# facebookresearch/D3GA

Hardware: AMD Instinct MI355X
Metric: fwd+bwd frames/sec @500k Gaussians 1920x1080 (higher is better)
Workload: dtype f32

## Files before the change

d3ga_amd/csrc/raster_pre.hip:

```cpp
#include "composite_common.h"
#include "raster_pre_body.h"

namespace d3ga {

constexpr int kShRow = 52;
constexpr int kShSlab = 64 * kShRow;
constexpr size_t kShLdsBytes = (size_t)(kBlock / 64) * kShSlab * sizeof(float);

__host__ __device__ __forceinline__ bool sh_staged(int M) { return M > 0 && (3 * M) % 4 == 0 && 3 * M <= 48; }

__device__ __forceinline__ void sh_slab_load(float *slab, const float *__restrict__ src, int rows, int M3, int lane) {
    const int nvec = rows * M3 / 4;
    for (int v = lane; v < nvec; v += 64) {
        const float4 x = reinterpret_cast<const float4 *>(src)[v];
        const int e = 4 * v, r = e / M3, c = e - r * M3;
        *reinterpret_cast<float4 *>(slab + r * kShRow + c) = x;
    }
}
__device__ __forceinline__ void sh_slab_store(const float *slab, float *__restrict__ dst, int rows, int M3, int lane) {
    const int nvec = rows * M3 / 4;
    for (int v = lane; v < nvec; v += 64) {
        const int e = 4 * v, r = e / M3, c = e - r * M3;
        reinterpret_cast<float4 *>(dst)[v] = *reinterpret_cast<const float4 *>(slab + r * kShRow + c);
    }
}

template <int ROWS>
struct ShRegs { float4 v[ROWS * 12 / 64]; };
template <int ROWS>
__device__ __forceinline__ ShRegs<ROWS> sh_rows48_load(const float *__restrict__ src, int lane) {
    ShRegs<ROWS> r;
#pragma unroll
    for (int k = 0; k < ROWS * 12 / 64; ++k) r.v[k] = reinterpret_cast<const float4 *>(src)[lane + 64 * k];
    return r;
}
template <int ROWS>
__device__ __forceinline__ void sh_rows48_to_slab(float *slab, const ShRegs<ROWS> &r, int lane) {
#pragma unroll
    for (int k = 0; k < ROWS * 12 / 64; ++k) {
        const int e = 4 * (lane + 64 * k), row = e / 48, c = e - row * 48;
        *reinterpret_cast<float4 *>(slab + row * kShRow + c) = r.v[k];
    }
}
template <int ROWS>
__device__ __forceinline__ void sh_rows48_store(const float *slab, float *__restrict__ dst, int lane) {
#pragma unroll
    for (int k = 0; k < ROWS * 12 / 64; ++k) {
        const int e = 4 * (lane + 64 * k), row = e / 48, c = e - row * 48;
        reinterpret_cast<float4 *>(dst)[lane + 64 * k] = *reinterpret_cast<const float4 *>(slab + row * kShRow + c);
    }
}

constexpr int kShPassRows = 32;
constexpr int kShHalfSlab = kShPassRows * kShRow;
constexpr size_t kShHalfLdsBytes = (size_t)(kBlock / 64) * kShHalfSlab * sizeof(float);

template <bool WANT_J>
__device__ __forceinline__ void staged_sh_colour(const d3ga_raster_params &prm, const float *__restrict__ means3D,
                                                 const float *__restrict__ shs, const float *__restrict__ campos,
                                                 float *s_sh, float acc[3], ShColJ &cj) {
    const int tid = threadIdx.x, lane = tid & 63, wave = tid >> 6;
    const int i = blockIdx.x * kBlock + tid;
    const int M3 = 3 * prm.M;
    float *slab = s_sh + wave * kShHalfSlab;
    const int row0 = blockIdx.x * kBlock + wave * 64;
    const int rows = min(64, prm.P - row0);
    const int nb = (prm.sh_degree + 1) * (prm.sh_degree + 1);
    float B[16];
    float dx = 0.f, dy = 0.f, dz = 1.f;
    if (WANT_J && i < prm.P) sh_view_dir(means3D, i, campos, dx, dy, dz);
    auto eval = [&](const float *row) __attribute__((always_inline)) {
        if (WANT_J) cj = sh_accumulate_jacobian(B, dx, dy, dz, row, nb, cj);
        else sh_accumulate(B, row, 0, 16, nb, acc);
    };
    if (M3 == 48 && rows == 64) {
        const float *src = shs + (size_t)48 * row0;
        const ShRegs<kShPassRows> h0 = sh_rows48_load<kShPassRows>(src, lane);
        const ShRegs<kShPassRows> h1 = sh_rows48_load<kShPassRows>(src + 48 * kShPassRows, lane);
        sh_view_basis(prm, means3D, i, campos, B);
        __builtin_amdgcn_wave_barrier();
        sh_rows48_to_slab<kShPassRows>(slab, h0, lane);
        __builtin_amdgcn_wave_barrier();
        if (lane / kShPassRows == 0) eval(slab + (lane % kShPassRows) * kShRow);
        __builtin_amdgcn_wave_barrier();
        sh_rows48_to_slab<kShPassRows>(slab, h1, lane);
        __builtin_amdgcn_wave_barrier();
        if (lane / kShPassRows == 1) eval(slab + (lane % kShPassRows) * kShRow);
        return;
    }
    if (i < prm.P) sh_view_basis(prm, means3D, i, campos, B);
    for (int h = 0; h < 2; ++h) {
        const int r = min(kShPassRows, rows - kShPassRows * h);
        __builtin_amdgcn_wave_barrier();
        if (r > 0) sh_slab_load(slab, shs + (size_t)M3 * (row0 + kShPassRows * h), r, M3, lane);
        __builtin_amdgcn_wave_barrier();
        if (i < prm.P && lane / kShPassRows == h) eval(slab + (lane % kShPassRows) * kShRow);
    }
}

struct TileRect { bool visible; int r0, r1, r2, r3; };
__device__ __forceinline__ TileRect view_tile_rect(const PreOut &o, int tile_row0) {
    const Splat &sp = o.sp;
    return TileRect{sp.visible, sp.rect[0], sp.rect[1] + tile_row0, sp.rect[2], sp.rect[3] + tile_row0};
}
__device__ __forceinline__ void write_geom_records(const GeomBuf &geom, int i, const PreOut &o, bool keep_cov, int tile_row0,
                                                   int32_t *__restrict__ radii, bool want_j, const ShColJ &cj) {
    const Splat &sp = o.sp;
    if (keep_cov) {
#pragma unroll
        for (int k = 0; k < 6; ++k) geom.cov3D[6 * (size_t)i + k] = o.c6[k];
    }
    radii[i] = sp.radius;
    geom.depth[i] = sp.depth;
    geom.rect[i] = sp.visible ? make_uint2((uint32_t)sp.rect[0] | ((uint32_t)(sp.rect[1] + tile_row0) << 16),
                                           (uint32_t)sp.rect[2] | ((uint32_t)(sp.rect[3] + tile_row0) << 16))
                              : make_uint2(0u, 0u);
    geom.conic_o[i] = make_float4(sp.conic[0], sp.conic[1], sp.conic[2], o.opacity);
    {
        const SplatCull sc = splat_cull(sp.conic[0], sp.conic[1], sp.conic[2], o.opacity);
        geom.xyh[i] = make_float4(sp.px, sp.py, sp.visible ? sc.hx : -1.0f, sc.hy);
    }
    geom.rgb_invd[i] = make_float4(o.rgb[0], o.rgb[1], o.rgb[2], sp.visible ? 1.0f / sp.depth : 0.f);
    geom.clamped[i] = o.clampmask;
    if (want_j) dcol_store(geom.dcol, geom.dcol_stride, i, cj);
}

__device__ __forceinline__ PreOut window_clip(PreOut o, int x0, int y0, int gx, int gy) {
    Splat &sp = o.sp;
    const int r0 = max(sp.rect[0], x0) - x0, r1 = max(sp.rect[1], y0) - y0;
    const int r2 = min(sp.rect[2], x0 + gx) - x0, r3 = min(sp.rect[3], y0 + gy) - y0;
    if (sp.visible && r2 > r0 && r3 > r1) { sp.rect[0] = r0; sp.rect[1] = r1; sp.rect[2] = r2; sp.rect[3] = r3; }
    else { sp.visible = false; sp.rect[0] = sp.rect[1] = sp.rect[2] = sp.rect[3] = 0; }
    return o;
}
__global__ void window_table_kernel(d3ga_raster_params prm, const float *__restrict__ campos, int views, int4 *__restrict__ table) {
    const int v = blockIdx.x * blockDim.x + threadIdx.x;
    if (v >= views) return;
    const ViewCam c = view_cam(prm, nullptr, nullptr, campos + (size_t)D3GA_CAMERA_SLOT_WINDOWED_FLOATS * v, true);
    table[v] = make_int4(c.ox, c.oy, c.W, c.H);
}

struct TileResv { TileWindow win; uint32_t base[kResvSlots]; };
__device__ __forceinline__ TileResv tile_reserve_issue(uint32_t *s_win, const TileRect &t, int gx, uint32_t *__restrict__ tile_count,
                                                       uint32_t *__restrict__ tile_count2, uint32_t *__restrict__ vis_part) {
    const int lane = threadIdx.x & 63;
    TileResv r;
    r.win = wave_tile_window(t.visible, t.r0, t.r1, t.r2, t.r3);
#pragma unroll
    for (int j = 0; j < kResvSlots; ++j) r.base[j] = 0u;
    const unsigned long long vis = __ballot(t.visible);
    if (lane == 0 && vis) atomicAdd(&vis_part[((blockIdx.x * (kBlock / 64) + (threadIdx.x >> 6)) % kVisParts) * kVisStride], (uint32_t)__popcll(vis));
    if (r.win.empty()) return r;
    if (r.win.fits()) {
        const int area = r.win.area();
        __builtin_amdgcn_wave_barrier();
#pragma unroll
        for (int j = 0; j < kResvSlots; ++j)
            if (lane + 64 * j < area) s_win[lane + 64 * j] = 0u;
        __builtin_amdgcn_wave_barrier();
        if (t.visible)
            for (int ty = t.r1; ty < t.r3; ++ty)
                for (int tx = t.r0; tx < t.r2; ++tx) atomicAdd(&s_win[(ty - r.win.y0) * r.win.w + (tx - r.win.x0)], 1u);
        __builtin_amdgcn_wave_barrier();
        const float inv_w = 1.0f / (float)r.win.w;
#pragma unroll
        for (int j = 0; j < kResvSlots; ++j) {
            const int k = lane + 64 * j;
            const uint32_t c = k < area ? s_win[k] : 0u;
            if (c) r.base[j] = atomicAdd(&tile_count[r.win.tile_of(k, gx, inv_w)], c);
        }
    } else {
        if (lane == 0) atomicOr(&vis_part[kUnresvWord], 1u);
        if (t.visible)
            for (int ty = t.r1; ty < t.r3; ++ty)
                for (int tx = t.r0; tx < t.r2; ++tx) atomicAdd(&tile_count2[ty * gx + tx], 1u);
    }
    return r;
}
__device__ __forceinline__ void tile_reserve_store(const TileResv &r, uint32_t *__restrict__ rec) {
    const int lane = threadIdx.x & 63;
    if (lane == 0)
        *reinterpret_cast<uint4 *>(rec) = make_uint4((uint32_t)r.win.x0 | ((uint32_t)r.win.y0 << 16), (uint32_t)r.win.w | ((uint32_t)r.win.h << 16), 0u, 0u);
    if (r.win.empty() || !r.win.fits()) return;
    const int area = r.win.area();
#pragma unroll
    for (int j = 0; j < kResvSlots; ++j)
        if (lane + 64 * j < area) rec[kResvHdr + lane + 64 * j] = r.base[j];
}

template <bool WIN>
__device__ __forceinline__ PreOut preprocess_view(const d3ga_raster_params &prm, const ViewCam &cam, int i, const float *means3D,
                                                    const float *sh_row, bool staged, const ShColJ &cj, bool pre, const float (&pc6)[6],
                                                    float pop, const float *colors_precomp, const float *opacities, const float *scales,
                                                    const float *rotations, const float *cov3D_precomp, int gx, int gy) {
    PreLoaded pl;
    pl.has_sh = staged; pl.has_c6 = pre;
    pl.sh[0] = cj.a0; pl.sh[1] = cj.a1; pl.sh[2] = cj.a2;
#pragma unroll
    for (int k = 0; k < 6; ++k) pl.c6[k] = pc6[k];
    pl.op = pop;
    PreOut o = preprocess_one(prm, cam, i, means3D, sh_row, colors_precomp, opacities, scales, rotations, cov3D_precomp, pl);
    if constexpr (WIN) o = window_clip(o, cam.ox / kTile, cam.oy / kTile, gx, gy);
    return o;
}

template <bool WANT_J, bool WIN>
__global__ __launch_bounds__(kBlock) void preprocess_kernel(
    d3ga_raster_params prm, const float *__restrict__ means3D, const float *__restrict__ shs,
    const float *__restrict__ colors_precomp, const float *__restrict__ opacities, const float *__restrict__ scales,
    const float *__restrict__ rotations, const float *__restrict__ cov3D_precomp, const float *__restrict__ viewmatrix,
    const float *__restrict__ projmatrix, const float *__restrict__ campos, GeomBuf geom,
    uint32_t *__restrict__ tile_count, uint32_t *__restrict__ tile_count2, uint32_t *__restrict__ vis_part,
    uint32_t *__restrict__ resv , int32_t *__restrict__ radii,
    int tile_row0 ) {
    const ViewCam cam = view_cam(prm, viewmatrix, projmatrix, campos, WIN);
    const int gx = (prm.W + kTile - 1) / kTile + (WIN ? 1 : 0), gy = (prm.H + kTile - 1) / kTile + 1;
    extern __shared__ __attribute__((aligned(16))) char smem[];
    float *s_sh = reinterpret_cast<float *>(smem);
    const int tid = threadIdx.x, wave = tid >> 6;
    const int i = blockIdx.x * kBlock + tid;
    const int M3 = 3 * prm.M;
    const bool staged = shs != nullptr && sh_staged(prm.M);
    uint32_t *s_win = reinterpret_cast<uint32_t *>(smem) + wave * (staged ? kShHalfSlab : kResvStride);
    float pc6[6] = {0.f, 0.f, 0.f, 0.f, 0.f, 0.f}, pop = 0.f;
    const bool pre = staged && cov3D_precomp != nullptr;
    if (pre && i < prm.P) {
#pragma unroll
        for (int k = 0; k < 6; ++k) pc6[k] = cov3D_precomp[6 * (size_t)i + k];
        pop = opacities[i];
    }
    ShColJ cj = {0.f, 0.f, 0.f, 0.f, 0.f, 0.f, 0.f, 0.f, 0.f, 0.f, 0.f, 0.f};
    float acc[3] = {0.f, 0.f, 0.f};
    if (staged) {
        staged_sh_colour<WANT_J>(prm, means3D, shs, campos, s_sh, acc, cj);
        if (!WANT_J) { cj.a0 = acc[0]; cj.a1 = acc[1]; cj.a2 = acc[2]; }
    }
    TileRect tr = {false, 0, 0, 0, 0};
    PreOut o = {};
    if (i < prm.P) {
        o = staged ? preprocess_view<WIN>(prm, cam, i, means3D, nullptr, true, cj, pre, pc6, pop, colors_precomp, opacities, scales,
                                          rotations, cov3D_precomp, gx, gy)
                   : preprocess_view<WIN>(prm, cam, i, means3D, shs ? shs + (size_t)M3 * i : nullptr, false, cj, false, pc6, pop,
                                          colors_precomp, opacities, scales, rotations, cov3D_precomp, gx, gy);
        tr = view_tile_rect(o, tile_row0);
    }
    const TileResv rs = tile_reserve_issue(s_win, tr, gx, tile_count, tile_count2, vis_part);
    if (i < prm.P) write_geom_records(geom, i, o, !cov3D_precomp, tile_row0, radii, WANT_J, cj);
    tile_reserve_store(rs, resv + (size_t)(blockIdx.x * (kBlock / 64) + wave) * kResvStride);
}

template <bool WANT_J, int KV>
__device__ __forceinline__ void staged_sh_colour_views(const d3ga_raster_params &prm, const float *__restrict__ means3D, size_t pv,
                                                       const float *__restrict__ shs, const ViewCams<KV> &cams, float *s_sh,
                                                       ShColJ (&cj)[KV]) {
    const int tid = threadIdx.x, lane = tid & 63, wave = tid >> 6;
    const int i = blockIdx.x * kBlock + tid;
    const int M3 = 3 * prm.M;
    float *slab = s_sh + wave * kShHalfSlab;
    const int row0 = blockIdx.x * kBlock + wave * 64;
    const int rows = min(64, prm.P - row0);
    const int nb = (prm.sh_degree + 1) * (prm.sh_degree + 1);
    auto eval = [&](const float *row) __attribute__((always_inline)) {
#pragma unroll
        for (int v = 0; v < KV; ++v) {
            float B[16];
            const float *mv = means3D + 3 * pv * v;
            if (WANT_J) {
                float dx, dy, dz;
                sh_view_dir(mv, i, cams.cp[v], dx, dy, dz);
                sh_basis(prm.sh_degree, dx, dy, dz, B);
                cj[v] = sh_accumulate_jacobian(B, dx, dy, dz, row, nb, cj[v]);
            } else {
                sh_view_basis(prm, mv, i, cams.cp[v], B);
                float acc[3] = {cj[v].a0, cj[v].a1, cj[v].a2};
                sh_accumulate(B, row, 0, 16, nb, acc);
                cj[v].a0 = acc[0]; cj[v].a1 = acc[1]; cj[v].a2 = acc[2];
            }
        }
    };
    if (M3 == 48 && rows == 64) {
        const float *src = shs + (size_t)48 * row0;
        const ShRegs<kShPassRows> h0 = sh_rows48_load<kShPassRows>(src, lane);
        const ShRegs<kShPassRows> h1 = sh_rows48_load<kShPassRows>(src + 48 * kShPassRows, lane);
        __builtin_amdgcn_wave_barrier();
        sh_rows48_to_slab<kShPassRows>(slab, h0, lane);
        __builtin_amdgcn_wave_barrier();
        if (lane / kShPassRows == 0) eval(slab + (lane % kShPassRows) * kShRow);
        __builtin_amdgcn_wave_barrier();
        sh_rows48_to_slab<kShPassRows>(slab, h1, lane);
        __builtin_amdgcn_wave_barrier();
        if (lane / kShPassRows == 1) eval(slab + (lane % kShPassRows) * kShRow);
        return;
    }
    for (int h = 0; h < 2; ++h) {
        const int r = min(kShPassRows, rows - kShPassRows * h);
        __builtin_amdgcn_wave_barrier();
        if (r > 0) sh_slab_load(slab, shs + (size_t)M3 * (row0 + kShPassRows * h), r, M3, lane);
        __builtin_amdgcn_wave_barrier();
        if (i < prm.P && lane / kShPassRows == h) eval(slab + (lane % kShPassRows) * kShRow);
    }
}

template <bool WANT_J, int KV>
__global__ __launch_bounds__(kBlock) void preprocess_views_kernel(
    d3ga_raster_params prm, const float *__restrict__ means3D, const float *__restrict__ shs,
    const float *__restrict__ colors_precomp, const float *__restrict__ opacities, const float *__restrict__ scales,
    const float *__restrict__ rotations, const float *__restrict__ cov3D_precomp, ViewCams<KV> cams, GeomBuf geom ,
    uint32_t *__restrict__ tile_count, uint32_t *__restrict__ tile_count2, uint32_t *__restrict__ vis_part,
    uint32_t *__restrict__ resv , int32_t *__restrict__ radii ,
    int tile_row0, int gyv, size_t pv ) {
    extern __shared__ __attribute__((aligned(16))) char smem[];
    float *s_sh = reinterpret_cast<float *>(smem);
    const int tid = threadIdx.x, wave = tid >> 6;
    const int i = blockIdx.x * kBlock + tid;
    uint32_t *s_win = reinterpret_cast<uint32_t *>(smem) + wave * kShHalfSlab;
    const size_t wpv = (size_t)gridDim.x * (kBlock / 64);
    float pc6[6] = {0.f, 0.f, 0.f, 0.f, 0.f, 0.f}, pop = 0.f;
    const bool pre = cov3D_precomp != nullptr && pv == 0;
    if (pre && i < prm.P) {
#pragma unroll
        for (int k = 0; k < 6; ++k) pc6[k] = cov3D_precomp[6 * (size_t)i + k];
        pop = opacities[i];
    }
    ShColJ cj[KV];
#pragma unroll
    for (int v = 0; v < KV; ++v) cj[v] = ShColJ{0.f, 0.f, 0.f, 0.f, 0.f, 0.f, 0.f, 0.f, 0.f, 0.f, 0.f, 0.f};
    staged_sh_colour_views<WANT_J, KV>(prm, means3D, pv, shs, cams, s_sh, cj);
    const int gx = (prm.W + kTile - 1) / kTile;
#pragma unroll
    for (int v = 0; v < KV; ++v) {
        TileRect tr = {false, 0, 0, 0, 0};
        PreOut o = {};
        if (i < prm.P) {
            const size_t og = pv * v;
            o = preprocess_view<false>(prm, view_cam(prm, cams.vm[v], cams.pm[v], cams.cp[v], false), i, means3D + 3 * og, nullptr, true,
                                       cj[v], pre, pc6, pop, colors_precomp, opacities, scales ? scales + 3 * og : nullptr,
                                       rotations ? rotations + 4 * og : nullptr, cov3D_precomp ? cov3D_precomp + 6 * og : nullptr, gx, 0);
            tr = view_tile_rect(o, tile_row0 + v * gyv);
        }
        const TileResv rs = tile_reserve_issue(s_win, tr, gx, tile_count, tile_count2, vis_part);
        if (i < prm.P)
            write_geom_records(geom_view(geom, prm.P, v), i, o, !cov3D_precomp, tile_row0 + v * gyv, radii + (size_t)prm.P * v, WANT_J, cj[v]);
        tile_reserve_store(rs, resv + (wpv * v + blockIdx.x * (kBlock / 64) + wave) * kResvStride);
    }
}

template <bool WANT_J>
__global__ __launch_bounds__(kBlock) void recolor_kernel(d3ga_raster_params prm, const float *__restrict__ means3D,
                                                         const float *__restrict__ shs,
                                                         const float *__restrict__ colors_precomp,
                                                         const float *__restrict__ campos, GeomBuf src, GeomBuf dst) {
    extern __shared__ __attribute__((aligned(16))) char smem[];
    float *s_sh = reinterpret_cast<float *>(smem);
    const int i = blockIdx.x * kBlock + threadIdx.x;
    const int M3 = 3 * prm.M;
    const bool staged = shs != nullptr && sh_staged(prm.M);
    ShColJ cj = {0.f, 0.f, 0.f, 0.f, 0.f, 0.f, 0.f, 0.f, 0.f, 0.f, 0.f, 0.f};
    float acc[3] = {0.f, 0.f, 0.f};
    if (staged) staged_sh_colour<WANT_J>(prm, means3D, shs, campos, s_sh, acc, cj);
    if (i >= prm.P) return;
    if (WANT_J) {
        acc[0] = cj.a0; acc[1] = cj.a1; acc[2] = cj.a2;
        dcol_store(dst.dcol, dst.dcol_stride, i, cj);
    }
    const uint2 rc = src.rect[i];
    const bool visible = rect_visible(rc.x, rc.y);
    const float depth = src.depth[i];
    dst.depth[i] = depth;
    dst.conic_o[i] = src.conic_o[i];
    dst.xyh[i] = src.xyh[i];
    dst.rect[i] = rc;
#pragma unroll
    for (int k = 0; k < 6; ++k) dst.cov3D[6 * (size_t)i + k] = src.cov3D[6 * (size_t)i + k];
    float rgb[3] = {0.f, 0.f, 0.f};
    uint8_t mask = 0;
    if (visible) {
        if (colors_precomp) {
            rgb[0] = colors_precomp[3 * (size_t)i]; rgb[1] = colors_precomp[3 * (size_t)i + 1];
            rgb[2] = colors_precomp[3 * (size_t)i + 2];
        } else {
            if (!staged) {
                float B[16];
                sh_view_basis(prm, means3D, i, campos, B);
                sh_accumulate(B, shs + (size_t)M3 * i, 0, 16, (prm.sh_degree + 1) * (prm.sh_degree + 1), acc);
            }
#pragma unroll
            for (int c = 0; c < 3; ++c) {
                const float v = acc[c] + 0.5f;
                if (v < 0.f) mask |= (uint8_t)(1u << c);
                rgb[c] = fmaxf(v, 0.f);
            }
        }
    }
    dst.rgb_invd[i] = make_float4(rgb[0], rgb[1], rgb[2], visible ? 1.0f / depth : 0.f);
    dst.clamped[i] = mask;
}

__device__ __forceinline__ ViewRecs view_recs(const GeomBuf &g, const float *acc) {
    return ViewRecs{reinterpret_cast<const uint32_t *>(g.rect), acc, g.clamped, reinterpret_cast<const float *>(g.conic_o), g.dcol,
                    g.dcol_stride};
}

template <bool WIN>
__global__ __launch_bounds__(kBlock) void preprocess_bwd_kernel(
    d3ga_raster_params prm, const float *__restrict__ means3D, const float *__restrict__ shs,
    const float *__restrict__ scales, const float *__restrict__ rotations, const float *__restrict__ viewmatrix,
    const float *__restrict__ projmatrix, const float *__restrict__ campos, GeomBuf geom,
    const float *__restrict__ acc, float *__restrict__ dL_dmeans3D, float *__restrict__ dL_dmeans2D,
    float *__restrict__ dL_dopacity, float *__restrict__ dL_dsh, float *__restrict__ dL_dcolors,
    float *__restrict__ dL_dcov3D, float *__restrict__ dL_dscales, float *__restrict__ dL_drots,
    const float *__restrict__ cov3D_precomp, int accum ) {
    const ViewCam cam = view_cam(prm, viewmatrix, projmatrix, campos, WIN);
    extern __shared__ __attribute__((aligned(16))) char smem[];
    float *s_sh = reinterpret_cast<float *>(smem);
    const int tid = threadIdx.x, lane = tid & 63, wave = tid >> 6;
    const int i = blockIdx.x * kBlock + tid;
    const int M3 = 3 * prm.M;
    const bool staged = shs != nullptr && sh_staged(prm.M);
    const int row0 = blockIdx.x * kBlock + wave * 64;
    const int rows = min(64, prm.P - row0);
    float *slab = s_sh + wave * kShSlab;
    const bool full48 = M3 == 48 && rows == 64;
    uint2 rc = make_uint2(0u, 0u);
    AccRec ar;
    float c6[6] = {0.f, 0.f, 0.f, 0.f, 0.f, 0.f};
    uint8_t clampmask = 0;
    float act_opacity = 0.f;
    if (i < prm.P) {
        rc = geom.rect[i];
        ar = acc_load(acc, i, prm.acc_self_clearing);
#pragma unroll
        for (int k = 0; k < 6; ++k) c6[k] = (cov3D_precomp ? cov3D_precomp : geom.cov3D)[6 * (size_t)i + k];
        clampmask = geom.clamped[i];
        act_opacity = geom.conic_o[i].w;
    }
    const bool have_j = staged && !prm.forward_only;
    ShColJ jd = {0.f, 0.f, 0.f, 0.f, 0.f, 0.f, 0.f, 0.f, 0.f, 0.f, 0.f, 0.f};
    if (have_j && i < prm.P) jd = dcol_load(geom.dcol, geom.dcol_stride, i);
    if (staged && !have_j) {
        if (full48) sh_rows48_to_slab<64>(slab, sh_rows48_load<64>(shs + (size_t)48 * row0, lane), lane);
        else if (rows > 0) sh_slab_load(slab, shs + (size_t)M3 * row0, rows, M3, lane);
        __builtin_amdgcn_wave_barrier();
// ... 318 lines not shown
```

d3ga_amd/csrc/raster_pre_body.h:

```cpp
#pragma once
#include "../../include/d3ga.h"
#include "d3ga_math.h"

namespace d3ga {

D3GA_HD V3 ld3(const float *p, size_t i) { return v3(p[3 * i], p[3 * i + 1], p[3 * i + 2]); }

struct PreOut {
    Splat sp;
    float c6[6];
    float rgb[3];
    float opacity;
    uint8_t clampmask;
};

D3GA_HD void sh_view_dir(const float *means3D, int i, const float *campos, float &x, float &y, float &z) {
    D3GA_NO_CONTRACT
    const V3 m = ld3(means3D, i);
    const float dx = m.x - campos[0], dy = m.y - campos[1], dz = m.z - campos[2];
    const float inv = 1.0f / sqrtf(dx * dx + dy * dy + dz * dz);
    x = dx * inv; y = dy * inv; z = dz * inv;
}
D3GA_HD void sh_view_basis(const d3ga_raster_params &prm, const float *means3D, int i, const float *campos, float B[16]) {
    float x, y, z;
    sh_view_dir(means3D, i, campos, x, y, z);
    sh_basis(prm.sh_degree, x, y, z, B);
}
struct ShColJ { float a0, a1, a2, j0, j1, j2, j3, j4, j5, j6, j7, j8; };
D3GA_HD ShColJ sh_accumulate_jacobian(const float B[16], float x, float y, float z, const float *row, int nb, ShColJ o) {
    const float xx = x * x, yy = y * y, zz = z * z, xy = x * y, yz = y * z, xz = x * z;
    o.j0 = o.j1 = o.j2 = o.j3 = o.j4 = o.j5 = o.j6 = o.j7 = o.j8 = 0.f;
#define D3GA_SHJ(K, GX, GY, GZ)                                                                             \
    if (K < nb) {                                                                                           \
        const float r0 = row[3 * K], r1 = row[3 * K + 1], r2 = row[3 * K + 2];                              \
        o.a0 = fmaf(B[K], r0, o.a0); o.a1 = fmaf(B[K], r1, o.a1); o.a2 = fmaf(B[K], r2, o.a2);                                               \
        const float gx_ = (GX), gy_ = (GY), gz_ = (GZ);                                                     \
        o.j0 += gx_ * r0; o.j1 += gx_ * r1; o.j2 += gx_ * r2;                                               \
        o.j3 += gy_ * r0; o.j4 += gy_ * r1; o.j5 += gy_ * r2;                                               \
        o.j6 += gz_ * r0; o.j7 += gz_ * r1; o.j8 += gz_ * r2;                                               \
    }
    if (0 < nb) { o.a0 = fmaf(B[0], row[0], o.a0); o.a1 = fmaf(B[0], row[1], o.a1); o.a2 = fmaf(B[0], row[2], o.a2); }
    D3GA_SHJ(1, 0.f, -kC1, 0.f)
    D3GA_SHJ(2, 0.f, 0.f, kC1)
    D3GA_SHJ(3, -kC1, 0.f, 0.f)
    D3GA_SHJ(4, kC2_0 * y, kC2_0 * x, 0.f)
    D3GA_SHJ(5, 0.f, kC2_1 * z, kC2_1 * y)
    D3GA_SHJ(6, -2.f * kC2_2 * x, -2.f * kC2_2 * y, 4.f * kC2_2 * z)
    D3GA_SHJ(7, kC2_3 * z, 0.f, kC2_3 * x)
    D3GA_SHJ(8, 2.f * kC2_4 * x, -2.f * kC2_4 * y, 0.f)
    D3GA_SHJ(9, kC3_0 * 6.f * xy, kC3_0 * 3.f * (xx - yy), 0.f)
    D3GA_SHJ(10, kC3_1 * yz, kC3_1 * xz, kC3_1 * xy)
    D3GA_SHJ(11, kC3_2 * -2.f * xy, kC3_2 * (4.f * zz - xx - 3.f * yy), kC3_2 * 8.f * yz)
    D3GA_SHJ(12, kC3_3 * -6.f * xz, kC3_3 * -6.f * yz, kC3_3 * 3.f * (2.f * zz - xx - yy))
    D3GA_SHJ(13, kC3_4 * (4.f * zz - 3.f * xx - yy), kC3_4 * -2.f * xy, kC3_4 * 8.f * xz)
    D3GA_SHJ(14, kC3_5 * 2.f * xz, kC3_5 * -2.f * yz, kC3_5 * (xx - yy))
    D3GA_SHJ(15, kC3_6 * 3.f * (xx - yy), kC3_6 * -6.f * xy, 0.f)
#undef D3GA_SHJ
    return o;
}
D3GA_HD void sh_accumulate(const float B[16], const float *part, int k0, int k1, int nb, float acc[3]) {
#pragma unroll
    for (int k = 0; k < 16; ++k) {
        if (k >= k0 && k < k1 && k < nb) {
            const float *c = part + 3 * (k - k0);
            acc[0] = fmaf(B[k], c[0], acc[0]); acc[1] = fmaf(B[k], c[1], acc[1]); acc[2] = fmaf(B[k], c[2], acc[2]);
        }
    }
}

struct ViewCam {
    const float *vm, *pm, *cp;
    float tanfovx, tanfovy;
    int W, H;
    int ox, oy;
};
D3GA_HD ViewCam view_cam(const d3ga_raster_params &prm, const float *vm, const float *pm, const float *cp, bool win) {
    ViewCam c = {vm, pm, cp, prm.tanfovx, prm.tanfovy, prm.W, prm.H, 0, 0};
    if (!(prm.tanfovx > 0.f)) { c.tanfovx = cp[3]; c.tanfovy = cp[4]; }
    if (win) { c.W = (int)cp[5]; c.H = (int)cp[6]; c.ox = (int)cp[7]; c.oy = (int)cp[8]; }
    return c;
}
template <int K>
struct ViewCams { const float *vm[K], *pm[K], *cp[K]; };

D3GA_HD bool rect_visible(uint32_t lo, uint32_t hi) { return ((hi & 0xffffu) > (lo & 0xffffu)) && ((hi >> 16) > (lo >> 16)); }
struct AccRec { float a[12]; };
D3GA_HD AccRec acc_load(const float *acc, size_t j, bool self_clearing) {
    float *p = (float *)__builtin_assume_aligned(const_cast<float *>(acc) + D3GA_ACC_STRIDE * j, 64);
    AccRec r;
    uint32_t any = 0;
    for (int k = 0; k < 12; ++k) { r.a[k] = p[k]; any |= __builtin_bit_cast(uint32_t, r.a[k]); }
    if (self_clearing && any)
        for (int k = 0; k < 12; ++k) p[k] = 0.f;
    return r;
}
D3GA_HD ShColJ dcol_load(const float *dcol, int64_t stride, size_t j) {
    ShColJ c = {0.f, 0.f, 0.f, 0.f, 0.f, 0.f, 0.f, 0.f, 0.f, 0.f, 0.f, 0.f};
    c.j0 = dcol[j]; c.j1 = dcol[stride + j]; c.j2 = dcol[2 * stride + j];
    c.j3 = dcol[3 * stride + j]; c.j4 = dcol[4 * stride + j]; c.j5 = dcol[5 * stride + j];
    c.j6 = dcol[6 * stride + j]; c.j7 = dcol[7 * stride + j]; c.j8 = dcol[8 * stride + j];
    return c;
}
D3GA_HD void dcol_store(float *dcol, int64_t stride, size_t j, const ShColJ &c) {
    dcol[j] = c.j0; dcol[stride + j] = c.j1; dcol[2 * stride + j] = c.j2;
    dcol[3 * stride + j] = c.j3; dcol[4 * stride + j] = c.j4; dcol[5 * stride + j] = c.j5;
    dcol[6 * stride + j] = c.j6; dcol[7 * stride + j] = c.j7; dcol[8 * stride + j] = c.j8;
}

struct PreLoaded {
    bool has_sh = false, has_c6 = false;
    float sh[3] = {0.f, 0.f, 0.f};
    float c6[6] = {0.f, 0.f, 0.f, 0.f, 0.f, 0.f};
    float op = 0.f;
};
D3GA_HD PreOut preprocess_one(const d3ga_raster_params &prm, const ViewCam &cam, int i, const float *means3D, const float *sh_row,
                              const float *colors_precomp, const float *opacities, const float *scales,
                              const float *rotations, const float *cov3D_precomp, const PreLoaded pl = PreLoaded()) {
    PreOut o;
    const V3 mean = ld3(means3D, i);
    const float raw_opacity = pl.has_c6 ? pl.op : opacities[i];
    if (pl.has_c6) {
        for (int k = 0; k < 6; ++k) o.c6[k] = pl.c6[k];
    } else if (cov3D_precomp) {
        for (int k = 0; k < 6; ++k) o.c6[k] = cov3D_precomp[6 * (size_t)i + k];
    } else {
        const float s[3] = {scales[3 * (size_t)i], scales[3 * (size_t)i + 1], scales[3 * (size_t)i + 2]};
        const float q[4] = {rotations[4 * (size_t)i], rotations[4 * (size_t)i + 1], rotations[4 * (size_t)i + 2],
                            rotations[4 * (size_t)i + 3]};
        cov3d_from_scale_rot(s, prm.scale_modifier, q, o.c6);
    }
    o.sp = project_gaussian(mean, o.c6, cam.vm, cam.pm, cam.W, cam.H, cam.tanfovx, cam.tanfovy, prm.antialiasing != 0);
    o.rgb[0] = o.rgb[1] = o.rgb[2] = 0.f;
    o.clampmask = 0;
    o.opacity = 0.f;
    if (!o.sp.visible) return o;
    o.opacity = raw_opacity;
    if (prm.opacity_activation == D3GA_OPACITY_SIGMOID) o.opacity = 1.0f / (1.0f + expf(-o.opacity));
    if (!(o.opacity == o.opacity)) {
        o.sp.visible = false; o.sp.radius = 0;
        o.sp.rect[0] = o.sp.rect[1] = o.sp.rect[2] = o.sp.rect[3] = 0;
        o.opacity = 0.f;
        return o;
    }
    o.opacity *= o.sp.aa;
    if (colors_precomp) {
        o.rgb[0] = colors_precomp[3 * (size_t)i]; o.rgb[1] = colors_precomp[3 * (size_t)i + 1];
        o.rgb[2] = colors_precomp[3 * (size_t)i + 2];
    } else {
        float acc[3] = {0.f, 0.f, 0.f};
        if (pl.has_sh) {
            acc[0] = pl.sh[0]; acc[1] = pl.sh[1]; acc[2] = pl.sh[2];
        } else {
            float B[16];
            sh_view_basis(prm, means3D, i, cam.cp, B);
            sh_accumulate(B, sh_row, 0, 16, (prm.sh_degree + 1) * (prm.sh_degree + 1), acc);
        }
        for (int c = 0; c < 3; ++c) {
            const float v = acc[c] + 0.5f;
            if (v < 0.f) o.clampmask |= (uint8_t)(1u << c);
            o.rgb[c] = fmaxf(v, 0.f);
        }
    }
    return o;
}

D3GA_HD PreOut preprocess_one(const d3ga_raster_params &prm, int i, const float *means3D, const float *sh_row,
                              const float *colors_precomp, const float *opacities, const float *scales,
                              const float *rotations, const float *cov3D_precomp, const float *viewmatrix,
                              const float *projmatrix, const float *campos, const PreLoaded pl = PreLoaded()) {
    const ViewCam cam = {viewmatrix, projmatrix, campos, prm.tanfovx, prm.tanfovy, prm.W, prm.H, 0, 0};
    return preprocess_one(prm, cam, i, means3D, sh_row, colors_precomp, opacities, scales, rotations, cov3D_precomp, pl);
}

struct BwdView { float gmean[3], g6[6], gr[3], B[16], gop; };
D3GA_HD BwdView preprocess_bwd_view(const d3ga_raster_params &prm, const ViewCam &cam, bool visible, V3 mean, const float *c6,
                                    const float *a, uint8_t clampmask, float act_opacity, bool sh, bool have_j, ShColJ jd,
                                    const float *sh_row, float *dsh_row = nullptr) {
    BwdView r;
    float gmean[3] = {0.f, 0.f, 0.f}, g6[6] = {0.f, 0.f, 0.f, 0.f, 0.f, 0.f};
    r.gr[0] = r.gr[1] = r.gr[2] = 0.f;
    float aa = 1.0f;
    if (visible) {
        cov2d_bwd(mean, c6, cam.vm, cam.W, cam.H, cam.tanfovx, cam.tanfovy, a[3], a[4], a[5], g6, gmean,
                  prm.antialiasing != 0, a[6], act_opacity, &aa);
        project_bwd(mean, cam.pm, a[0], a[1], gmean);
        const float *vm = cam.vm;
        const float z = vm[2] * mean.x + vm[6] * mean.y + vm[10] * mean.z + vm[14];
        const float gz = -a[10] / (z * z);
        gmean[0] += vm[2] * gz; gmean[1] += vm[6] * gz; gmean[2] += vm[10] * gz;
    }
    if (sh && visible) {
        r.gr[0] = (clampmask & 1) ? 0.f : a[7]; r.gr[1] = (clampmask & 2) ? 0.f : a[8]; r.gr[2] = (clampmask & 4) ? 0.f : a[9];
        const float *gr = r.gr;
        float B[16];
        const V3 d0 = mean - v3(cam.cp[0], cam.cp[1], cam.cp[2]);
        const float inv = 1.0f / sqrtf(dot(d0, d0));
        const float x = d0.x * inv, y = d0.y * inv, z = d0.z * inv;
        sh_basis(prm.sh_degree, x, y, z, B);
        const int nb = (prm.sh_degree + 1) * (prm.sh_degree + 1), nbM = prm.M;
        float *out = dsh_row;
        V3 gd = v3(0.f, 0.f, 0.f);
        if (have_j) {
            gd = v3(jd.j0 * gr[0] + jd.j1 * gr[1] + jd.j2 * gr[2], jd.j3 * gr[0] + jd.j4 * gr[1] + jd.j5 * gr[2],
                    jd.j6 * gr[0] + jd.j7 * gr[1] + jd.j8 * gr[2]);
#pragma unroll
            for (int k = 0; k < 16; ++k) {
                if (k < nb) { if (out) { out[3 * k] = B[k] * gr[0]; out[3 * k + 1] = B[k] * gr[1]; out[3 * k + 2] = B[k] * gr[2]; } }
                else if (k < nbM && out) { out[3 * k] = 0.f; out[3 * k + 1] = 0.f; out[3 * k + 2] = 0.f; }
            }
        } else {
            float Bx[16], By[16], Bz[16];
            sh_basis_grad(prm.sh_degree, x, y, z, Bx, By, Bz);
            const float *sh = sh_row;
#pragma unroll
            for (int k = 0; k < 16; ++k) {
                if (k < nb) {
                    const float s0 = sh[3 * k], s1 = sh[3 * k + 1], s2 = sh[3 * k + 2];
                    if (out) { out[3 * k] = B[k] * gr[0]; out[3 * k + 1] = B[k] * gr[1]; out[3 * k + 2] = B[k] * gr[2]; }
                    const float w = s0 * gr[0] + s1 * gr[1] + s2 * gr[2];
                    gd.x += Bx[k] * w; gd.y += By[k] * w; gd.z += Bz[k] * w;
                } else if (k < nbM && out) {
                    out[3 * k] = 0.f; out[3 * k + 1] = 0.f; out[3 * k + 2] = 0.f;
                }
            }
        }
        const V3 gm = normalize_bwd(d0, gd);
        gmean[0] += gm.x; gmean[1] += gm.y; gmean[2] += gm.z;
        for (int k = 0; k < 16; ++k) r.B[k] = B[k];
    }
    const float op = act_opacity / aa, g_op = a[6] * aa;
    for (int k = 0; k < 3; ++k) r.gmean[k] = gmean[k];
    for (int k = 0; k < 6; ++k) r.g6[k] = g6[k];
    r.gop = prm.opacity_activation == D3GA_OPACITY_SIGMOID ? g_op * op * (1.0f - op) : g_op;
    return r;
}

D3GA_HD void preprocess_bwd_one(const d3ga_raster_params &prm, const ViewCam &cam, int i, bool visible, const float *means3D,
                                const float *sh_row, const float *scales, const float *rotations,
                                const float *c6, uint8_t clampmask, const float *a, float *dL_dmeans3D,
                                float *dL_dmeans2D, float *dL_dopacity, float *dsh_row, float *dL_dcolors,
                                float *dL_dcov3D, float *dL_dscales, float *dL_drots, float act_opacity = 0.f,
                                bool have_j = false, ShColJ jd = ShColJ(), int accum = 0) {
    const BwdView r = preprocess_bwd_view(prm, cam, visible, ld3(means3D, i), c6, a, clampmask, act_opacity, sh_row != nullptr,
                                          have_j, jd, sh_row, dsh_row);
    if (sh_row) {
// ... 147 lines not shown
```

Baseline: 2703.

## Overlap SH row loads with projection and tile reservation in full-wavefront preprocess

Adds a specialised full-wavefront preprocess path for the 48-float SH, precomputed-covariance, Jacobian case. It issues the first half of each SH slab load, then runs projection, tile reservation and geometry record writes while those loads are in flight, and only afterwards evaluates colour from LDS. It also loads each mean once and passes it by value instead of reloading it from global memory, and makes the wave tile window scalar via readfirstlane. The intent is to hide global-load latency behind the projection math and to cut redundant loads. The cost is higher register pressure from live float4 loads held across the projection work, plus a more complex split of the geom and colour paths.

Measured after the change: 2739, median of 6. +1.3%, better.

```diff
diff --git a/d3ga_amd/csrc/raster_pre.hip b/d3ga_amd/csrc/raster_pre.hip
--- a/d3ga_amd/csrc/raster_pre.hip
+++ b/d3ga_amd/csrc/raster_pre.hip
@@ -55,10 +55,37 @@
 constexpr int kShHalfSlab = kShPassRows * kShRow;
 constexpr size_t kShHalfLdsBytes = (size_t)(kBlock / 64) * kShHalfSlab * sizeof(float);
 
+#define D3GA_SH_HALF_ISSUE(H, SRC)                                                                                        \
+    const float4 *H##g = reinterpret_cast<const float4 *>(SRC) + lane;                                                     \
+    const float4 H##0 = H##g[0], H##1 = H##g[64], H##2 = H##g[128], H##3 = H##g[192], H##4 = H##g[256], H##5 = H##g[320];
+#define D3GA_SH_HALF_TO_SLAB(H)                                                                                           \
+    sh_row48_put(slab, lane, H##0); sh_row48_put(slab, lane + 64, H##1); sh_row48_put(slab, lane + 128, H##2);             \
+    sh_row48_put(slab, lane + 192, H##3); sh_row48_put(slab, lane + 256, H##4); sh_row48_put(slab, lane + 320, H##5);
+static_assert(kShPassRows * 12 / 64 == 6, "six 16-byte loads per lane and half");
+__device__ __forceinline__ void sh_row48_put(float *slab, int v, float4 x) {
+    const int e = 4 * v, row = e / 48, c = e - row * 48;
+    *reinterpret_cast<float4 *>(slab + row * kShRow + c) = x;
+}
+template <class Before, class Eval>
+__device__ __forceinline__ void sh_two_pass48(float *slab, const float *__restrict__ src, int lane, Before &&before, Eval &&eval) {
+    D3GA_SH_HALF_ISSUE(h0_, src)
+    before();
+    __builtin_amdgcn_wave_barrier();
+    D3GA_SH_HALF_TO_SLAB(h0_)
+    __builtin_amdgcn_wave_barrier();
+    if (lane / kShPassRows == 0) eval(slab + (lane % kShPassRows) * kShRow);
+    D3GA_SH_HALF_ISSUE(h1_, src + 48 * kShPassRows)
+    __builtin_amdgcn_wave_barrier();
+    D3GA_SH_HALF_TO_SLAB(h1_)
+    __builtin_amdgcn_wave_barrier();
+    if (lane / kShPassRows == 1) eval(slab + (lane % kShPassRows) * kShRow);
+}
+#undef D3GA_SH_HALF_ISSUE
+#undef D3GA_SH_HALF_TO_SLAB
+
 template <bool WANT_J>
-__device__ __forceinline__ void staged_sh_colour(const d3ga_raster_params &prm, const float *__restrict__ means3D,
-                                                 const float *__restrict__ shs, const float *__restrict__ campos,
-                                                 float *s_sh, float acc[3], ShColJ &cj) {
+__device__ __forceinline__ void staged_sh_colour(const d3ga_raster_params &prm, V3 mean, const float *__restrict__ shs,
+                                                 const float *__restrict__ campos, float *s_sh, float acc[3], ShColJ &cj) {
     const int tid = threadIdx.x, lane = tid & 63, wave = tid >> 6;
     const int i = blockIdx.x * kBlock + tid;
     const int M3 = 3 * prm.M;
@@ -68,16 +95,22 @@
     const int nb = (prm.sh_degree + 1) * (prm.sh_degree + 1);
     float B[16];
     float dx = 0.f, dy = 0.f, dz = 1.f;
-    if (WANT_J && i < prm.P) sh_view_dir(means3D, i, campos, dx, dy, dz);
     auto eval = [&](const float *row) __attribute__((always_inline)) {
         if (WANT_J) cj = sh_accumulate_jacobian(B, dx, dy, dz, row, nb, cj);
         else sh_accumulate(B, row, 0, 16, nb, acc);
     };
     if (M3 == 48 && rows == 64) {
+        if (WANT_J) {
+            sh_two_pass48(slab, shs + (size_t)48 * row0, lane, [&]() __attribute__((always_inline)) {
+                sh_view_dir(mean, campos, dx, dy, dz);
+                sh_basis(prm.sh_degree, dx, dy, dz, B);
+            }, eval);
+            return;
+        }
         const float *src = shs + (size_t)48 * row0;
         const ShRegs<kShPassRows> h0 = sh_rows48_load<kShPassRows>(src, lane);
         const ShRegs<kShPassRows> h1 = sh_rows48_load<kShPassRows>(src + 48 * kShPassRows, lane);
-        sh_view_basis(prm, means3D, i, campos, B);
+        sh_view_basis(prm, mean, campos, B);
         __builtin_amdgcn_wave_barrier();
         sh_rows48_to_slab<kShPassRows>(slab, h0, lane);
         __builtin_amdgcn_wave_barrier();
@@ -88,7 +121,8 @@
         if (lane / kShPassRows == 1) eval(slab + (lane % kShPassRows) * kShRow);
         return;
     }
-    if (i < prm.P) sh_view_basis(prm, means3D, i, campos, B);
+    if (WANT_J && i < prm.P) sh_view_dir(mean, campos, dx, dy, dz);
+    if (i < prm.P) sh_view_basis(prm, mean, campos, B);
     for (int h = 0; h < 2; ++h) {
         const int r = min(kShPassRows, rows - kShPassRows * h);
         __builtin_amdgcn_wave_barrier();
@@ -103,8 +137,8 @@
     const Splat &sp = o.sp;
     return TileRect{sp.visible, sp.rect[0], sp.rect[1] + tile_row0, sp.rect[2], sp.rect[3] + tile_row0};
 }
-__device__ __forceinline__ void write_geom_records(const GeomBuf &geom, int i, const PreOut &o, bool keep_cov, int tile_row0,
-                                                   int32_t *__restrict__ radii, bool want_j, const ShColJ &cj) {
+__device__ __forceinline__ float write_geom_records_splat(const GeomBuf &geom, int i, const PreOut &o, bool keep_cov, int tile_row0,
+                                                          int32_t *__restrict__ radii) {
     const Splat &sp = o.sp;
     if (keep_cov) {
 #pragma unroll
@@ -120,9 +154,18 @@
         const SplatCull sc = splat_cull(sp.conic[0], sp.conic[1], sp.conic[2], o.opacity);
         geom.xyh[i] = make_float4(sp.px, sp.py, sp.visible ? sc.hx : -1.0f, sc.hy);
     }
-    geom.rgb_invd[i] = make_float4(o.rgb[0], o.rgb[1], o.rgb[2], sp.visible ? 1.0f / sp.depth : 0.f);
-    geom.clamped[i] = o.clampmask;
+    return sp.visible ? 1.0f / sp.depth : 0.f;
+}
+__device__ __forceinline__ void write_geom_records_colour(const GeomBuf &geom, int i, float r, float g, float b, float invd,
+                                                           uint8_t clampmask, bool want_j, const ShColJ &cj) {
+    geom.rgb_invd[i] = make_float4(r, g, b, invd);
+    geom.clamped[i] = clampmask;
     if (want_j) dcol_store(geom.dcol, geom.dcol_stride, i, cj);
+}
+__device__ __forceinline__ void write_geom_records(const GeomBuf &geom, int i, const PreOut &o, bool keep_cov, int tile_row0,
+                                                   int32_t *__restrict__ radii, bool want_j, const ShColJ &cj) {
+    const float invd = write_geom_records_splat(geom, i, o, keep_cov, tile_row0, radii);
+    write_geom_records_colour(geom, i, o.rgb[0], o.rgb[1], o.rgb[2], invd, o.clampmask, want_j, cj);
 }
 
 __device__ __forceinline__ PreOut window_clip(PreOut o, int x0, int y0, int gx, int gy) {
@@ -141,11 +184,16 @@
 }
 
 struct TileResv { TileWindow win; uint32_t base[kResvSlots]; };
+template <bool SCALAR_WIN = false >
 __device__ __forceinline__ TileResv tile_reserve_issue(uint32_t *s_win, const TileRect &t, int gx, uint32_t *__restrict__ tile_count,
                                                        uint32_t *__restrict__ tile_count2, uint32_t *__restrict__ vis_part) {
     const int lane = threadIdx.x & 63;
     TileResv r;
     r.win = wave_tile_window(t.visible, t.r0, t.r1, t.r2, t.r3);
+    if constexpr (SCALAR_WIN) {
+    r.win.x0 = __builtin_amdgcn_readfirstlane(r.win.x0); r.win.y0 = __builtin_amdgcn_readfirstlane(r.win.y0);
+    r.win.w = __builtin_amdgcn_readfirstlane(r.win.w); r.win.h = __builtin_amdgcn_readfirstlane(r.win.h);
+    }
 #pragma unroll
     for (int j = 0; j < kResvSlots; ++j) r.base[j] = 0u;
     const unsigned long long vis = __ballot(t.visible);
@@ -189,7 +237,7 @@
 }
 
 template <bool WIN>
-__device__ __forceinline__ PreOut preprocess_view(const d3ga_raster_params &prm, const ViewCam &cam, int i, const float *means3D,
+__device__ __forceinline__ PreOut preprocess_view(const d3ga_raster_params &prm, const ViewCam &cam, int i, V3 mean,
                                                     const float *sh_row, bool staged, const ShColJ &cj, bool pre, const float (&pc6)[6],
                                                     float pop, const float *colors_precomp, const float *opacities, const float *scales,
                                                     const float *rotations, const float *cov3D_precomp, int gx, int gy) {
@@ -199,9 +247,52 @@
 #pragma unroll
     for (int k = 0; k < 6; ++k) pl.c6[k] = pc6[k];
     pl.op = pop;
-    PreOut o = preprocess_one(prm, cam, i, means3D, sh_row, colors_precomp, opacities, scales, rotations, cov3D_precomp, pl);
+    pl.has_mean = true; pl.mean = mean;
+    PreOut o = preprocess_one(prm, cam, i, nullptr, sh_row, colors_precomp, opacities, scales, rotations, cov3D_precomp, pl);
     if constexpr (WIN) o = window_clip(o, cam.ox / kTile, cam.oy / kTile, gx, gy);
     return o;
+}
+
+template <bool WIN>
+__device__ __forceinline__ void preprocess_full_wavefront(
+    const d3ga_raster_params &prm, const ViewCam &cam, const float *__restrict__ means3D, const float *__restrict__ shs,
+    const float *__restrict__ opacities, const float *__restrict__ cov3D_precomp, const float *__restrict__ campos, const GeomBuf &geom,
+    uint32_t *__restrict__ tile_count,
+    uint32_t *__restrict__ tile_count2, uint32_t *__restrict__ vis_part, uint32_t *__restrict__ rec, int32_t *__restrict__ radii,
+    int tile_row0, int gx, int gy, float *slab) {
+    const int tid = threadIdx.x, lane = tid & 63;
+    const int i = blockIdx.x * kBlock + tid;
+    const int row0 = i - lane;
+    PreLoaded pl;
+    pl.has_sh = true; pl.has_c6 = true; pl.has_mean = true;
+    pl.mean = ld3(means3D, i);
+    pl.op = opacities[i];
+#pragma unroll
+    for (int k = 0; k < 6; ++k) pl.c6[k] = cov3D_precomp[6 * (size_t)i + k];
+    const int nb = (prm.sh_degree + 1) * (prm.sh_degree + 1);
+    float B[16];
+    float dx, dy, dz, invd;
+    bool visible = false;
+    TileResv rs;
+    ShColJ cj = {0.f, 0.f, 0.f, 0.f, 0.f, 0.f, 0.f, 0.f, 0.f, 0.f, 0.f, 0.f};
+    sh_two_pass48(slab, shs + (size_t)48 * row0, lane, [&]() __attribute__((always_inline)) {
+        PreOut o = preprocess_geom(prm, cam, i, pl.mean, opacities, nullptr, nullptr, cov3D_precomp, pl);
+        if constexpr (WIN) visible = o.sp.visible;
+        if constexpr (WIN) o = window_clip(o, cam.ox / kTile, cam.oy / kTile, gx, gy);
+        rs = tile_reserve_issue<true>(reinterpret_cast<uint32_t *>(slab), view_tile_rect(o, tile_row0), gx, tile_count, tile_count2, vis_part);
+        invd = write_geom_records_splat(geom, i, o, false, tile_row0, radii);
+        sh_view_dir(pl.mean, campos, dx, dy, dz);
+        sh_basis(prm.sh_degree, dx, dy, dz, B);
+    }, [&](const float *row) __attribute__((always_inline)) {
+        cj = sh_accumulate_jacobian(B, dx, dy, dz, row, nb, cj);
+    });
+    pl.sh[0] = cj.a0; pl.sh[1] = cj.a1; pl.sh[2] = cj.a2;
+    float rgb[3] = {0.f, 0.f, 0.f};
+    uint8_t clampmask = 0;
+    if constexpr (!WIN) visible = invd != 0.f;
+    preprocess_colour(prm, cam, i, pl.mean, nullptr, nullptr, pl, visible, rgb, clampmask);
+    write_geom_records_colour(geom, i, rgb[0], rgb[1], rgb[2], invd, clampmask, true, cj);
+    tile_reserve_store(rs, rec);
 }
 
 template <bool WANT_J, bool WIN>
@@ -222,31 +313,42 @@
     const int M3 = 3 * prm.M;
     const bool staged = shs != nullptr && sh_staged(prm.M);
     uint32_t *s_win = reinterpret_cast<uint32_t *>(smem) + wave * (staged ? kShHalfSlab : kResvStride);
+    uint32_t *const rec = resv + (size_t)(blockIdx.x * (kBlock / 64) + wave) * kResvStride;
+    const int row0 = blockIdx.x * kBlock + wave * 64;
+    if (WANT_J && staged && cov3D_precomp && M3 == 48 && prm.P - row0 >= 64) {
+        preprocess_full_wavefront<WIN>(prm, cam, means3D, shs, opacities, cov3D_precomp, campos, geom, tile_count, tile_count2, vis_part, rec,
+                                       radii, tile_row0, gx, gy, s_sh + wave * kShHalfSlab);
+        return;
+    }
+    V3 mean = v3(0.f, 0.f, 0.f);
     float pc6[6] = {0.f, 0.f, 0.f, 0.f, 0.f, 0.f}, pop = 0.f;
     const bool pre = staged && cov3D_precomp != nullptr;
-    if (pre && i < prm.P) {
-#pragma unroll
-        for (int k = 0; k < 6; ++k) pc6[k] = cov3D_precomp[6 * (size_t)i + k];
-        pop = opacities[i];
+    if (i < prm.P) {
+        mean = ld3(means3D, i);
+        if (pre) {
+#pragma unroll
+            for (int k = 0; k < 6; ++k) pc6[k] = cov3D_precomp[6 * (size_t)i + k];
+            pop = opacities[i];
+        }
     }
     ShColJ cj = {0.f, 0.f, 0.f, 0.f, 0.f, 0.f, 0.f, 0.f, 0.f, 0.f, 0.f, 0.f};
     float acc[3] = {0.f, 0.f, 0.f};
     if (staged) {
-        staged_sh_colour<WANT_J>(prm, means3D, shs, campos, s_sh, acc, cj);
+        staged_sh_colour<WANT_J>(prm, mean, shs, campos, s_sh, acc, cj);
         if (!WANT_J) { cj.a0 = acc[0]; cj.a1 = acc[1]; cj.a2 = acc[2]; }
     }
     TileRect tr = {false, 0, 0, 0, 0};
     PreOut o = {};
     if (i < prm.P) {
-        o = staged ? preprocess_view<WIN>(prm, cam, i, means3D, nullptr, true, cj, pre, pc6, pop, colors_precomp, opacities, scales,
+        o = staged ? preprocess_view<WIN>(prm, cam, i, mean, nullptr, true, cj, pre, pc6, pop, colors_precomp, opacities, scales,
                                           rotations, cov3D_precomp, gx, gy)
-                   : preprocess_view<WIN>(prm, cam, i, means3D, shs ? shs + (size_t)M3 * i : nullptr, false, cj, false, pc6, pop,
+                   : preprocess_view<WIN>(prm, cam, i, mean, shs ? shs + (size_t)M3 * i : nullptr, false, cj, false, pc6, pop,
                                           colors_precomp, opacities, scales, rotations, cov3D_precomp, gx, gy);
         tr = view_tile_rect(o, tile_row0);
     }
     const TileResv rs = tile_reserve_issue(s_win, tr, gx, tile_count, tile_count2, vis_part);
     if (i < prm.P) write_geom_records(geom, i, o, !cov3D_precomp, tile_row0, radii, WANT_J, cj);
-    tile_reserve_store(rs, resv + (size_t)(blockIdx.x * (kBlock / 64) + wave) * kResvStride);
+    tile_reserve_store(rs, rec);
 }
 
 template <bool WANT_J, int KV>
@@ -333,7 +435,7 @@
         PreOut o = {};
         if (i < prm.P) {
             const size_t og = pv * v;
-            o = preprocess_view<false>(prm, view_cam(prm, cams.vm[v], cams.pm[v], cams.cp[v], false), i, means3D + 3 * og, nullptr, true,
+            o = preprocess_view<false>(prm, view_cam(prm, cams.vm[v], cams.pm[v], cams.cp[v], false), i, ld3(means3D + 3 * og, i), nullptr, true,
                                        cj[v], pre, pc6, pop, colors_precomp, opacities, scales ? scales + 3 * og : nullptr,
                                        rotations ? rotations + 4 * og : nullptr, cov3D_precomp ? cov3D_precomp + 6 * og : nullptr, gx, 0);
             tr = view_tile_rect(o, tile_row0 + v * gyv);
@@ -357,7 +459,7 @@
     const bool staged = shs != nullptr && sh_staged(prm.M);
     ShColJ cj = {0.f, 0.f, 0.f, 0.f, 0.f, 0.f, 0.f, 0.f, 0.f, 0.f, 0.f, 0.f};
     float acc[3] = {0.f, 0.f, 0.f};
-    if (staged) staged_sh_colour<WANT_J>(prm, means3D, shs, campos, s_sh, acc, cj);
+    if (staged) staged_sh_colour<WANT_J>(prm, i < prm.P ? ld3(means3D, i) : v3(0.f, 0.f, 0.f), shs, campos, s_sh, acc, cj);
     if (i >= prm.P) return;
     if (WANT_J) {
         acc[0] = cj.a0; acc[1] = cj.a1; acc[2] = cj.a2;
diff --git a/d3ga_amd/csrc/raster_pre_body.h b/d3ga_amd/csrc/raster_pre_body.h
--- a/d3ga_amd/csrc/raster_pre_body.h
+++ b/d3ga_amd/csrc/raster_pre_body.h
@@ -14,17 +14,22 @@
     uint8_t clampmask;
 };
 
-D3GA_HD void sh_view_dir(const float *means3D, int i, const float *campos, float &x, float &y, float &z) {
+D3GA_HD void sh_view_dir(V3 m, const float *campos, float &x, float &y, float &z) {
     D3GA_NO_CONTRACT
-    const V3 m = ld3(means3D, i);
     const float dx = m.x - campos[0], dy = m.y - campos[1], dz = m.z - campos[2];
     const float inv = 1.0f / sqrtf(dx * dx + dy * dy + dz * dz);
     x = dx * inv; y = dy * inv; z = dz * inv;
 }
+D3GA_HD void sh_view_dir(const float *means3D, int i, const float *campos, float &x, float &y, float &z) {
+    sh_view_dir(ld3(means3D, i), campos, x, y, z);
+}
+D3GA_HD void sh_view_basis(const d3ga_raster_params &prm, V3 m, const float *campos, float B[16]) {
+    float x, y, z;
+    sh_view_dir(m, campos, x, y, z);
+    sh_basis(prm.sh_degree, x, y, z, B);
+}
 D3GA_HD void sh_view_basis(const d3ga_raster_params &prm, const float *means3D, int i, const float *campos, float B[16]) {
-    float x, y, z;
-    sh_view_dir(means3D, i, campos, x, y, z);
-    sh_basis(prm.sh_degree, x, y, z, B);
+    sh_view_basis(prm, ld3(means3D, i), campos, B);
 }
 struct ShColJ { float a0, a1, a2, j0, j1, j2, j3, j4, j5, j6, j7, j8; };
 D3GA_HD ShColJ sh_accumulate_jacobian(const float B[16], float x, float y, float z, const float *row, int nb, ShColJ o) {
@@ -109,15 +114,15 @@
 
 struct PreLoaded {
     bool has_sh = false, has_c6 = false;
+    bool has_mean = false;
     float sh[3] = {0.f, 0.f, 0.f};
     float c6[6] = {0.f, 0.f, 0.f, 0.f, 0.f, 0.f};
     float op = 0.f;
+    V3 mean = {0.f, 0.f, 0.f};
 };
-D3GA_HD PreOut preprocess_one(const d3ga_raster_params &prm, const ViewCam &cam, int i, const float *means3D, const float *sh_row,
-                              const float *colors_precomp, const float *opacities, const float *scales,
-                              const float *rotations, const float *cov3D_precomp, const PreLoaded pl = PreLoaded()) {
+D3GA_HD PreOut preprocess_geom(const d3ga_raster_params &prm, const ViewCam &cam, int i, V3 mean, const float *opacities,
+                               const float *scales, const float *rotations, const float *cov3D_precomp, const PreLoaded &pl) {
     PreOut o;
-    const V3 mean = ld3(means3D, i);
     const float raw_opacity = pl.has_c6 ? pl.op : opacities[i];
     if (pl.has_c6) {
         for (int k = 0; k < 6; ++k) o.c6[k] = pl.c6[k];
@@ -143,24 +148,36 @@
         return o;
     }
     o.opacity *= o.sp.aa;
+    return o;
+}
+D3GA_HD void preprocess_colour(const d3ga_raster_params &prm, const ViewCam &cam, int i, V3 mean, const float *sh_row,
+                               const float *colors_precomp, const PreLoaded &pl, bool visible, float (&rgb)[3], uint8_t &clampmask) {
+    if (!visible) return;
     if (colors_precomp) {
-        o.rgb[0] = colors_precomp[3 * (size_t)i]; o.rgb[1] = colors_precomp[3 * (size_t)i + 1];
-        o.rgb[2] = colors_precomp[3 * (size_t)i + 2];
+        rgb[0] = colors_precomp[3 * (size_t)i]; rgb[1] = colors_precomp[3 * (size_t)i + 1];
+        rgb[2] = colors_precomp[3 * (size_t)i + 2];
     } else {
         float acc[3] = {0.f, 0.f, 0.f};
         if (pl.has_sh) {
             acc[0] = pl.sh[0]; acc[1] = pl.sh[1]; acc[2] = pl.sh[2];
         } else {
             float B[16];
-            sh_view_basis(prm, means3D, i, cam.cp, B);
+            sh_view_basis(prm, mean, cam.cp, B);
             sh_accumulate(B, sh_row, 0, 16, (prm.sh_degree + 1) * (prm.sh_degree + 1), acc);
         }
         for (int c = 0; c < 3; ++c) {
             const float v = acc[c] + 0.5f;
-            if (v < 0.f) o.clampmask |= (uint8_t)(1u << c);
-            o.rgb[c] = fmaxf(v, 0.f);
-        }
-    }
+            if (v < 0.f) clampmask |= (uint8_t)(1u << c);
+            rgb[c] = fmaxf(v, 0.f);
+        }
+    }
+}
+D3GA_HD PreOut preprocess_one(const d3ga_raster_params &prm, const ViewCam &cam, int i, const float *means3D, const float *sh_row,
+                              const float *colors_precomp, const float *opacities, const float *scales,
+                              const float *rotations, const float *cov3D_precomp, const PreLoaded pl = PreLoaded()) {
+    const V3 mean = pl.has_mean ? pl.mean : ld3(means3D, i);
+    PreOut o = preprocess_geom(prm, cam, i, mean, opacities, scales, rotations, cov3D_precomp, pl);
+    preprocess_colour(prm, cam, i, mean, sh_row, colors_precomp, pl, o.sp.visible, o.rgb, o.clampmask);
     return o;
 }
 
```
